# sebcossu/yocto_raytracing

Measured on AMD Instinct MI355X. Metric: Mrays/sec + ms/frame, instance10000 1920×1080×64spp, 1/2/4/8 MI355X, higher is better.
Workload: dtype f32; 1 GPU; instance10000 1920x1080 8x8 spp, amb 0.1, one frame per step; scene=instance10000, width=1920, height=1080, spp=64, parallelism=single GPU, algorithm=wavefront

## Files before the change

__graft_entry__.py:

```python
from __future__ import annotations

import ctypes
import importlib
import sys
from pathlib import Path

ROOT = Path(__file__).resolve().parent
if str(ROOT) not in sys.path:
    sys.path.insert(0, str(ROOT))


def _build_module():
    import importlib.util

    spec = importlib.util.spec_from_file_location("yrt_build", ROOT / "yocto_raytracing_amd" / "build.py")
    mod = importlib.util.module_from_spec(spec)
    spec.loader.exec_module(mod)
    return mod


def _variants_tool():
    import importlib.util

    spec = importlib.util.spec_from_file_location("yrt_build_variants", ROOT / "tools" / "build_variants.py")
    mod = importlib.util.module_from_spec(spec)
    spec.loader.exec_module(mod)
    return mod


def build() -> None:
    b = _build_module()
    b.build_library()
    b.build_oracle()
    t = _variants_tool()
    t.main(t.test_specs(), default_library=False, verbose=False)
    importlib.import_module("yocto_raytracing_amd")


def _oracle():
    lib = ctypes.CDLL(str(ROOT / "oracle" / "liboracle.so"))
    lib.oracle_load.restype = ctypes.c_void_p
    lib.oracle_load.argtypes = [ctypes.c_char_p]
    lib.oracle_render_rows.restype = ctypes.c_longlong
    lib.oracle_render_rows.argtypes = [ctypes.c_void_p, ctypes.c_float, ctypes.c_int, ctypes.c_int,
                                       ctypes.c_int, ctypes.c_int, ctypes.c_int, ctypes.c_void_p,
                                       ctypes.c_int, ctypes.c_int, ctypes.c_int, ctypes.c_void_p,
                                       ctypes.c_void_p]
    return lib


def smoke() -> None:
    import numpy as np

    import yocto_raytracing_amd as yrt

    if yrt.device_count() < 1:
        raise RuntimeError("smoke: no GPU visible")
    scene_path = ROOT / "tests" / "golden" / "scenes" / "simple.yrtscene"
    scn = yrt.load_scene(str(scene_path))
    yrt.build_bvh(scn)
    res, s = 36, 2
    img, stats = yrt.raytrace(scn, (0.1, 0.1, 0.1), res, s, return_stats=True)

    lib = _oracle()
    o = lib.oracle_load(str(scene_path).encode())
    h, w = img.shape[:2]
    rows = np.arange(h, dtype=np.int32)
    ref = np.zeros_like(img)
    nrays = lib.oracle_render_rows(o, 0.1, 0, res, 0, s, 16, rows.ctypes.data, h, 0, w, ref.ctypes.data, None)
    diff = float(np.abs(img - ref).max())
    exact = float(np.mean(img.view(np.uint32) == ref.view(np.uint32)))
    if stats["rays"] != nrays or diff > 1e-5:
        raise RuntimeError(f"smoke: GPU/oracle mismatch rays {stats['rays']} vs {nrays}, max|diff| {diff}")
    print(f"smoke ok: {w}x{h}x{s * s} rays={nrays} bit-exact={exact:.4f} max|diff|={diff:.3g}")


if __name__ == "__main__":
    build()
    smoke()
```

yocto_raytracing_amd/csrc/wavefront.hip:

```cpp
#include <hip/hip_runtime.h>

#include <algorithm>
#include <cstdio>
#include <cstdlib>
#include <cstring>
#include <stdexcept>
#include <type_traits>

#include "item_magic.h"
#include "packet_trace.h"
#include "trace_common.h"
#include "wf_workspace.h"
#include "yrt_render.h"

namespace yrt {
namespace {

constexpr int WF_BLOCK = 256;
#ifndef YRT_PRIMARY_BLOCK
#define YRT_PRIMARY_BLOCK 64
#endif
#ifndef YRT_SHADOW_BLOCK
#define YRT_SHADOW_BLOCK 64
#endif
// ... 1920 lines not shown
                vec3f v;
                float vlen;
                normalize_len(ro - p, v, vlen);
                for (int li = 0; li < S.nlights; li++) {
                    if (OCC4 ? ((occ_bits >> li) & 1u) != 0u : ldb(B.occl + (size_t)li * B.capacity + idx) != 0) continue;
                    const f4* lr = S.lights + 6 * li;
                    float4 lrec[6];
                    ld_scalar<6>(lr, lrec);
                    frame3f lf = {xyz(lrec[0]), xyz(lrec[1]), xyz(lrec[2]), xyz(lrec[3])};
                    vec3f lp0 = xyz(lrec[4]), ke = xyz(lrec[5]);
                    vec3f tp = transform_point(lf, lp0 - p);
                    vec3f l, h;
                    float r, hlen;
                    normalize_len(tp, l, r);
                    normalize_len(v + l, h, hlen);
                    vec3f kd = kd0, ks = ks0;
                    if (kd_txt >= 0) kd = kd * tkd;
                    if (ks_txt >= 0) ks = ks * tks;
                    const vec3f ker = div3(ke, r * r);
                    vec3f ld = kd * ker;
                    vec3f ls = ks * ker;
                    if (kind == kind_lines) {
                        float prodnl = dot(nrm, l);
                        float prodnh = dot(nrm, h);
                        if (prodnl < 0.0f) prodnl *= -1;
                        if (prodnh < 0.0f) prodnh *= -1;
                        float sinnl = __builtin_sqrtf(1.0f - prodnl);
                        float sinnh = __builtin_sqrtf(1.0f - prodnh);
                        ld = ld * sinnl;
                        ls = ls * spec_pow(sinnh, ns, ls);
                    } else {
                        ld = ld * smax(0.0f, dot(nrm, l));
                        ls = ls * spec_pow(smax(0.0f, dot(nrm, h)), ns, ls);
                    }
                    c = c + (ld + ls);
                    cd = cd + ld;
                    cs = cs + ls;
                }
                pc = c, pd = cd, ps = cs, pla = la;
                if (!reflective) {
                    R = c + la;
                } else {
                    truncated++;
                    vec3f t = {0.0f * kr.x, 0.0f * kr.y, 0.0f * kr.z};
                    pr = t;
                    R = (c + t) + la;
                }
            }
        }
        if constexpr (FUSE) {
            auto put = [&](int k, const vec3f& val) {
                if (!(P.mask >> k & 1)) return;
                fused[(k * 3 + 0) * ROW + threadIdx.x] = val.x;
                fused[(k * 3 + 1) * ROW + threadIdx.x] = val.y;
                fused[(k * 3 + 2) * ROW + threadIdx.x] = val.z;
            };
            put(pass_direct, pc), put(pass_diffuse, pd), put(pass_specular, ps);
            put(pass_reflection, pr), put(pass_ambient, pla), put(pass_count, R);
            continue;
        }
    }
    }
    if (FUSE) {
        __syncthreads();
        const int ppb = SB / C.spp;
        for (int t = (int)threadIdx.x; t < 3 * pass_planes * ppb; t += SB) {
            const int px = t / (3 * pass_planes), r = t - 3 * pass_planes * px;
            const int k = r / 3, comp = r - 3 * k;
            if (!(P.mask >> k & 1)) continue;
            const int pl = (int)(blockIdx.x * SB / C.spp) + px;
            int lx, ly, i, j;
            const bool valid = pl < C.npix && pixel_of(A, C, C.pix0 + pl, lx, ly, i, j);
            if (pl < C.npix && lx < A.tile_w && ly < A.tile_h) {
                float v = 0.0f;
                if (valid) {
                    const float* row = fused + (k * 3 + comp) * ROW + px * C.spp;
                    float acc = 0.0f;
                    for (int q = 0; q < C.spp; q++) acc = acc + row[q];
                    v = acc / float(C.spp);
                }
                float* o = reinterpret_cast<float*>(P.out[k] + (size_t)ly * A.out_stride + lx);
                o[comp] = v;
                if (comp == 0) o[3] = valid ? 1.0f : 0.0f;
            }
        }
    }
    flush(counters, cnt_depth_truncated, truncated);
}

struct group_buffers {
    int nplanes;
    unsigned amb_mask;
    const int* tab;
    float4* out[group_planes];
    f4* smp[group_planes];
    f4* rec[group_planes];
};

constexpr int shade_group_waves = 5;
template <bool FUSE, int SB = WF_BLOCK, bool OCC4 = false>
__global__ __launch_bounds__(SB, shade_group_waves) void k_shade_groups(dev_scene_view S, dev_render_args A, int level,
                                                                        int nsamp_level0, int max_depth, wf_buffers B,
                                                                        group_buffers G, unsigned long long* counters,
                                                                        chunk_args C) {
    constexpr int ROW = SB + 1;
    __shared__ float fused[FUSE ? group_planes * 3 * ROW : 1];
    __shared__ int cmp_count[SB / 64], cmp_base[SB / 64];
    __shared__ srgb_table srgb_lds;
    const float* lut = stage_srgb<SB, true>(S, srgb_lds);
    work_counts wc;
    unsigned long long truncated = 0;
    float amb_x = A.amb[0], amb_y = A.amb[1], amb_z = A.amb[2];
    float cam_x = A.cam.ox, cam_y = A.cam.oy, cam_z = A.cam.oz;
    asm volatile("" : "+s"(amb_x), "+s"(amb_y), "+s"(amb_z), "+s"(cam_x), "+s"(cam_y), "+s"(cam_z));
    const vec3f amb = {amb_x, amb_y, amb_z};
    const vec3f cam_o = {cam_x, cam_y, cam_z};
    const int nplanes = G.nplanes;
    const int* order = G.tab + group_planes + 1;
    const int stride = gridDim.x * SB;
    const int gout = (int)(blockIdx.x % (unsigned)level_segments);
    const int nseg = FUSE ? 1 : level ? level_segments : 1;
    for (int g = 0; g < nseg; g++) {
    const int n = (!FUSE && level) ? *seg_counter(B.count, level, g) : nsamp_level0;
    const int nround = (n + stride - 1) / stride;
    for (int round = 0; round < nround; round++) {
        const int j = round * stride + blockIdx.x * SB + threadIdx.x;
        const int idx = FUSE ? j : g * B.seg + j;
        bool hit = false, write_r = false, spawn = false, reflective = false;
        vec3f p = {0, 0, 0}, nrm = {0, 0, 0}, v = {0, 0, 0}, dr = {0, 0, 0};
        vec3f kd = {0, 0, 0}, ks = {0, 0, 0}, kr = {0, 0, 0}, la = {0, 0, 0}, la0 = {0, 0, 0}, t = {0, 0, 0};
        float ns = 0.0f;
        int mat = 0, kind = 0;
        uint32_t occ_bits = 0;
        if (j < n) {
            const float4 s0 = ld4s(B.surf0 + idx);
            if constexpr (OCC4) {
#pragma unroll
                for (int q = 0; q < 4; q++) {
                    const int lq = q < S.nlights ? q : 0;
                    occ_bits |= (ldb(B.occl + (size_t)lq * B.capacity + idx) != 0u ? 1u : 0u) << q;
                }
            }
            const int info = sample_state(s0);
            write_r = info != -2;
            hit = info >= 0;
            if (hit) {
                const float4 ro4 =
                    (!FUSE && level) ? ld4(B.ray_o(level) + idx) : make_float4(cam_o.x, cam_o.y, cam_o.z, 0.0f);
                vec2f uv;
                {
                    const float4 s1 = ld4s(B.surf1 + idx);
                    p = xyz(s0), nrm = xyz(s1), uv = {s1.w, B.need_v ? lds1(B.surfv + idx) : 0.0f};
                    mat = info_mat(info), kind = info & 3;
                }
                const vec3f ro = xyz(ro4);
                const float4 m0 = ld4(S.mats + 4 * mat), m1 = ld4(S.mats + 4 * mat + 1);
                const float4 m2 = ld4(S.mats + 4 * mat + 2), m3 = ld4(S.mats + 4 * mat + 3);
                const vec3f kd0 = xyz(m0), ks0 = xyz(m1);
                kr = xyz(m2), ns = m0.w;
                const int kd_txt = ibits(m1.w), ks_txt = ibits(m2.w);
                reflective = ibits(m3.w) & mat_reflective;
                const vec3f zero = {0.0f, 0.0f, 0.0f};
                la = amb * kd0, la0 = zero * kd0;
                vec3f tkd = {1, 1, 1}, tks = {1, 1, 1};
                if (kd_txt >= 0) {
                    tkd = eval_texture<false>(S, kd_txt, uv, wc, lut);
                    la = la * tkd, la0 = la0 * tkd;
                }
                if (ks_txt >= 0) tks = eval_texture<false>(S, ks_txt, uv, wc, lut);
                kd = kd0, ks = ks0;
                if (kd_txt >= 0) kd = kd * tkd;
                if (ks_txt >= 0) ks = ks * tks;
                float vlen;
                normalize_len(ro - p, v, vlen);
                if (reflective) {
                    if (FUSE || level + 1 >= max_depth || level + 1 >= B.nlevels) {
                        truncated++;
                        t = {0.0f * kr.x, 0.0f * kr.y, 0.0f * kr.z};
                    } else {
                        spawn = true;
                        dr = (nrm * 2.0f * dot(nrm, v)) - v;
                        write_r = false;
                    }
                }
            }
        }
        for (int k = 0; k < nplanes; k++) {
            const int q0 = __builtin_amdgcn_readfirstlane(G.tab[k]), q1 = __builtin_amdgcn_readfirstlane(G.tab[k + 1]);
            const bool ambk = G.amb_mask >> k & 1;
            vec3f R = {0, 0, 0};
            if (hit) {
                vec3f c = {0.0f, 0.0f, 0.0f};
                for (int q = q0; q < q1; q++) {
                    const int li = __builtin_amdgcn_readfirstlane(order[q]);
                    if (OCC4 ? ((occ_bits >> li) & 1u) != 0u : ldb(B.occl + (size_t)li * B.capacity + idx) != 0) continue;
                    float4 lrec[6];
                    ld_scalar<6>(S.lights + 6 * li, lrec);
                    frame3f lf = {xyz(lrec[0]), xyz(lrec[1]), xyz(lrec[2]), xyz(lrec[3])};
                    vec3f lp0 = xyz(lrec[4]), ke = xyz(lrec[5]);
                    vec3f tp = transform_point(lf, lp0 - p);
                    vec3f l, h;
                    float r, hlen;
                    normalize_len(tp, l, r);
                    normalize_len(v + l, h, hlen);
                    const vec3f ker = div3(ke, r * r);
                    vec3f ld = kd * ker;
                    vec3f ls = ks * ker;
                    if (kind == kind_lines) {
                        float prodnl = dot(nrm, l);
                        float prodnh = dot(nrm, h);
                        if (prodnl < 0.0f) prodnl *= -1;
                        if (prodnh < 0.0f) prodnh *= -1;
                        float sinnl = __builtin_sqrtf(1.0f - prodnl);
                        float sinnh = __builtin_sqrtf(1.0f - prodnh);
                        ld = ld * sinnl;
                        ls = ls * spec_pow(sinnh, ns, ls);
                    } else {
                        ld = ld * smax(0.0f, dot(nrm, l));
                        ls = ls * spec_pow(smax(0.0f, dot(nrm, h)), ns, ls);
                    }
                    c = c + (ld + ls);
                }
                const vec3f lak = ambk ? la : la0;
                if (!reflective)
                    R = c + lak;
                else if (!spawn)
                    R = (c + t) + lak;
                else
                    G.rec[k][(size_t)level * B.capacity + idx] = {c.x, c.y, c.z, __int_as_float(mat)};
            }
            if constexpr (FUSE) {
                fused[(k * 3 + 0) * ROW + threadIdx.x] = R.x;
                fused[(k * 3 + 1) * ROW + threadIdx.x] = R.y;
                fused[(k * 3 + 2) * ROW + threadIdx.x] = R.z;
            } else if (write_r) {
                vec3f col = R;
                int lev = level, node = idx;
                while (lev > 0) {
                    const int parent = ibits(B.ray_o(lev)[node].w);
                    const float4 d = ld4(G.rec[k] + (size_t)(lev - 1) * B.capacity + parent);
                    const float4 pkr = ld4(S.mats + 4 * ibits(d.w) + 2);
                    vec3f cc = {d.x, d.y, d.z};
                    const vec3f tt = {col.x * pkr.x, col.y * pkr.y, col.z * pkr.z};
                    cc = cc + tt;
                    if (ambk) cc = cc + xyz(ld4(B.rec1(lev - 1) + parent));
                    col = cc, node = parent, lev--;
                }
                G.smp[k][node] = {col.x, col.y, col.z, 1.0f};
            }
        }
        if constexpr (FUSE) continue;
        const unsigned long long mask = __ballot(spawn);
        const int w = threadIdx.x >> 6, lane = threadIdx.x & 63;
        if (spawn) B.rec1(level)[idx] = {la.x, la.y, la.z, 0};
        if (lane == 0) cmp_count[w] = __popcll(mask);
        __syncthreads();
        if (threadIdx.x == 0) {
            int tot = 0;
            for (int q = 0; q < SB / 64; q++) tot += cmp_count[q];
            int acc = tot ? atomicAdd(seg_counter(B.count, level + 1, gout), tot) : 0;
            for (int q = 0; q < SB / 64; q++) cmp_base[q] = acc, acc += cmp_count[q];
        }
        __syncthreads();
        if (spawn) {
            const int slot = gout * B.seg + cmp_base[w] + __popcll(mask & ((1ull << lane) - 1));
            B.ray_o(level + 1)[slot] = {p.x, p.y, p.z, __int_as_float(idx)};
            B.ray_d(level + 1)[slot] = {dr.x, dr.y, dr.z, 0};
        }
    }
    }
    if (FUSE) {
        __syncthreads();
        const int ppb = SB / C.spp;
        for (int e = (int)threadIdx.x; e < 3 * nplanes * ppb; e += SB) {
            const int px = e / (3 * nplanes), r = e - 3 * nplanes * px;
            const int k = r / 3, comp = r - 3 * k;
            const int pl = (int)(blockIdx.x * SB / C.spp) + px;
            int lx, ly, i, j;
            const bool valid = pl < C.npix && pixel_of(A, C, C.pix0 + pl, lx, ly, i, j);
            if (pl < C.npix && lx < A.tile_w && ly < A.tile_h) {
                float val = 0.0f;
                if (valid) {
                    const float* row = fused + (k * 3 + comp) * ROW + px * C.spp;
                    float acc = 0.0f;
                    for (int q = 0; q < C.spp; q++) acc = acc + row[q];
                    val = acc / float(C.spp);
                }
                float* o = reinterpret_cast<float*>(G.out[k] + (size_t)ly * A.out_stride + lx);
                o[comp] = val;
                if (comp == 0) o[3] = valid ? 1.0f : 0.0f;
            }
        }
    }
    flush(counters, cnt_depth_truncated, truncated);
}

#if !defined(YRT_SHADOW_SHADE_FUSE)
#define YRT_SHADOW_SHADE_FUSE 1
#endif
#define YRT_SHADOW_SHADE_KERNEL (YRT_SHADOW_SHADE_FUSE && YRT_SHADOW_ITEM_LIGHTS)
#if !defined(YRT_LIGHT_CARRY)
#define YRT_LIGHT_CARRY 1
#endif
#if (YRT_SHADOW_SHADE_KERNEL)
__global__ __launch_bounds__(SP_BLOCK, YRT_SHADOW_WAVES) void k_shadow_shade_persist(dev_scene_view S,
                                                                                      dev_render_args A, int nsamp,
                                                                                      int nx, wf_buffers B,
                                                                                      unsigned long long* counters,
                                                                                      chunk_args C,
                                                                                      float4* __restrict__ out) {
    constexpr int WPB = SP_BLOCK / 64;
    constexpr unsigned RUN = YRT_SHADOW_ITEM_RUN;
    constexpr int CARRY = YRT_LIGHT_CARRY ? 4 : 0;
    __shared__ float4 wave_slab[WPB][CARRY ? CARRY : 1][64];
    __shared__ unsigned wave_truncated[WPB];
    __shared__ srgb_table srgb_lds;
    __shared__ struct {
        dev_render_args A;
        chunk_args C;
    } args;
    const float* lut = stage_srgb<SP_BLOCK, false>(S, srgb_lds);
    if (threadIdx.x == 0) args.A = A, args.C = C;
    __syncthreads();
    float cam_x = A.cam.ox, cam_y = A.cam.oy, cam_z = A.cam.oz;
    asm volatile("" : "+s"(cam_x), "+s"(cam_y), "+s"(cam_z));
    const vec3f cam_o = {cam_x, cam_y, cam_z};
    const int nl = S.nlights;
    __builtin_assume(nl > 0);
    const unsigned n_items = (unsigned)nx;
    auto lane_now = []() {
        unsigned l;
        asm volatile("v_mbcnt_lo_u32_b32 %0, -1, 0\n\tv_mbcnt_hi_u32_b32 %0, -1, %0" : "=v"(l));
        return l;
    };
    const int w = __builtin_amdgcn_readfirstlane((int)(threadIdx.x >> 6));
    const unsigned xcd = blockIdx.x % 8u;
    unsigned rays = 0, culled = 0;
    if (lane_now() == 0) wave_truncated[w] = 0;
    constexpr unsigned CS = YRT_SHADOW_BLOCK_CHUNK;
    __shared__ chunk_ring ring;
    const unsigned head = head_items<RUN, CS>(n_items);
    chunk_ring_init<CS>(ring, B.queue + xcd, B.queue + 8, head / 8u);
    for (;;) {
        const unsigned q = chunk_ring_next<CS>(ring, B.queue + xcd, lane_now(), B.queue + 8, head / 8u);
        const unsigned it = split_item<RUN>(q, xcd, n_items, head);
        if (it >= n_items) break;
        const int bx = (int)it;
        uint32_t occ_bits = 0;
        for (int li = 0; li < nl; li++) {
            bool valid;
            const bool occ = shadow_item_light<0, true, true>(S, B, nsamp, bx, li, nl, lane_now(), cam_o, nullptr, rays,
                                                              culled, valid, li < CARRY ? wave_slab[w][li] : nullptr);
            occ_bits |= (occ ? 1u : 0u) << li;
        }
        const int idx = bx * 64 + (int)lane_now();
        vec3f R = {0, 0, 0};
        unsigned long long truncated = 0;
        if (idx < nsamp) {
            const float4 s0 = ld4(B.surf0 + idx);
            const int info = sample_state(s0);
            if (info >= 0) {
                const float4 ro4 = make_float4(cam_o.x, cam_o.y, cam_o.z, 0.0f);
                const float* amb = args.A.amb;
                work_counts wc;
                vec3f p = {0, 0, 0}, dr = {0, 0, 0}, rec_d = {0, 0, 0}, rec_la = {0, 0, 0};
                int rec_mat = 0;
                bool spawn = false, write_r = true;
                shade_hit<false, true, true, true>(S, B, idx, info, s0, ro4, occ_bits, 0, 1, amb, lut, wc, truncated, R, p,
                                             spawn, dr, rec_d, rec_la, rec_mat, write_r, (no_terms*)nullptr,
                                             CARRY ? &wave_slab[w][0][lane_now()] : nullptr, CARRY);
            }
        }
        const unsigned lane = lane_now();
        const unsigned ntrunc = (unsigned)__popcll(ballot(truncated != 0));
        if (ntrunc && lane == 0) wave_truncated[w] += ntrunc;
        wave_slab[w][0][lane] = make_float4(R.x, R.y, R.z, 1.0f);
        asm volatile("s_waitcnt lgkmcnt(0)" ::: "memory");
        const int spp = __builtin_amdgcn_readfirstlane(args.C.spp);
        if (spp == 64) {
            sum_pixels<64, 64>(args.A, args.C, out, wave_slab[w][0], bx, 1, (int)lane);
        } else {
            const int sl = __builtin_ctz((unsigned)spp);
            sum_pixels<64>(args.A, args.C, out, wave_slab[w][0], bx << (6 - sl), 64 >> sl, (int)lane);
        }
        asm volatile("s_waitcnt lgkmcnt(0)" ::: "memory");
    }
    const unsigned lane = lane_now();
    const unsigned long long first = lane == 0 ? 1ull : 0ull;
    flush_block_at<3, SP_BLOCK>(
        counters, {first * rays, first * culled, first * (lane == 0 ? wave_truncated[w] : 0u)},
        (unsigned)w * 64u + lane,
        [](unsigned k) { return k == 0 ? cnt_shadow_rays : k == 1 ? cnt_shadow_culled : cnt_depth_truncated; });
}
#endif

constexpr int AQ = 8;
template <class SMP, class OUT>
__device__ __forceinline__ void accumulate_plane(dev_render_args A, chunk_args C, SMP&& samples, OUT&& out) {
    __shared__ float4 stage[WF_BLOCK / 64][64 * (AQ + 1)];
    const int w = threadIdx.x >> 6, lane = threadIdx.x & 63;
    const int pl0 = blockIdx.x * WF_BLOCK + w * 64;
    const int np = max(0, min(64, C.npix - pl0));
    float4* S = stage[w];
    const f4* base = samples() + (size_t)pl0 * C.spp;
    vec3f acc = {0, 0, 0};
    for (int q0 = 0; q0 < C.spp; q0 += AQ) {
        const int qn = min(AQ, C.spp - q0);
        for (int e = lane; e < np * qn; e += 64) {
            const int px = e / qn, q = e % qn;
            S[px * (AQ + 1) + q] = ld4(base + (size_t)px * C.spp + q0 + q);
        }
        __syncthreads();
        if (lane < np)
            for (int q = 0; q < qn; q++) {
                const float4 c = S[lane * (AQ + 1) + q];
                acc = {acc.x + c.x, acc.y + c.y, acc.z + c.z};
            }
        __syncthreads();
    }
    if (lane >= np) return;
    const int pl = pl0 + lane;
    int lx, ly, i, j;
    const bool valid = pixel_of(A, C, C.pix0 + pl, lx, ly, i, j);
    if (lx >= A.tile_w || ly >= A.tile_h) return;
    const float d = float(C.spp);
    out()[(size_t)ly * A.out_stride + lx] =
        valid ? make_float4(acc.x / d, acc.y / d, acc.z / d, 1.0f) : make_float4(0.0f, 0.0f, 0.0f, 0.0f);
}

__global__ __launch_bounds__(WF_BLOCK) void k_accumulate(dev_render_args A, chunk_args C, wf_buffers B,
                                                         float4* __restrict__ out) {
    accumulate_plane(A, C, [&] { return B.rad; }, [&] { return out; });
}

__global__ __launch_bounds__(WF_BLOCK) void k_accumulate_passes(dev_render_args A, chunk_args C, wf_buffers B,
                                                                pass_buffers P) {
    const int k = (int)blockIdx.y;
    if (!(P.mask >> k & 1)) return;
    accumulate_plane(A, C, [&] { return k == pass_count ? B.rad : P.smp[k]; }, [&] { return P.out[k]; });
}

__global__ __launch_bounds__(WF_BLOCK) void k_accumulate_groups(dev_render_args A, chunk_args C, group_buffers G) {
    const int k = (int)blockIdx.y;
    accumulate_plane(A, C, [&] { return G.smp[k]; }, [&] { return G.out[k]; });
}

wf_buffers carve(void* base, const workspace_shape& s, pass_buffers* P, group_buffers* G) {
    wf_buffers B = {};
    workspace_carver w(base);
    int pass = -1;
    walk_workspace(s, [&](wf_slab slab, int k, size_t bytes) {
        void* const p = w.take(bytes);
        switch (slab) {
            case slab_count: B.count = (int*)p; break;
            case slab_queue: B.queue = (unsigned*)p; break;
            case slab_lstats: B.lstats = (unsigned long long*)p; break;
            case slab_surf0: B.surf0 = (f4*)p; break;
            case slab_surf1: B.surf1 = (f4*)p; break;
            case slab_surfv: B.surfv = (float*)p; break;
            case slab_occl: B.occl = (unsigned char*)p; break;
            case slab_rad: B.rad = (f4*)p; break;
            case slab_pbox: B.pbox = (f4*)p; break;
            case slab_lcount: B.lcount = (int*)p; break;
            case slab_lskip: B.lskip = (int*)p; break;
            case slab_lists: B.lists = (f4*)p; break;
            case slab_slists: B.slists = (f4*)p; break;
            case slab_ccount: B.ccount = (int*)p; break;
            case slab_cskip: B.cskip = (int*)p; break;
            case slab_clist: B.clist = (f4*)p; break;
            case slab_ray_o: B.ray_o_ = (f4*)p; break;
            case slab_ray_d: B.ray_d_ = (f4*)p; break;
            case slab_rec0: B.rec0_ = (f4*)p; break;
            case slab_rec1: B.rec1_ = (f4*)p; break;
            case slab_pass_smp:
                do pass++;
                while (!(P->mask >> pass & 1));
                P->smp[pass] = (f4*)p;
                break;
            case slab_group_tab: G->tab = (const int*)p; break;
            case slab_group_smp: G->smp[k] = (f4*)p; break;
            case slab_group_rec: G->rec[k] = (f4*)p; break;
        }
    });
    if (G) G->smp[0] = B.rad, G->rec[0] = B.rec0_;
    B.capacity = s.cap;
    B.nlevels = s.nlevels;
    return B;
}


hipError_t clear_counters(unsigned long long* counters, hipStream_t stream) {
    return counters ? hipMemsetAsync(counters, 0, (size_t)cnt_slots * cnt_count * sizeof(unsigned long long), stream)
                    : hipSuccess;
}

template <class F>
long long chunk_target(const device_scene& ds, const dev_render_args& A, F&& bytes_of) {
    long long target = 1ll << (ds.reflective ? MIRROR_CHUNK_LOG2 : CHUNK_LOG2);
    if (bytes_of(target) > ds.work_bytes) {
        size_t free_b = 0, total_b = 0;
        if (hipMemGetInfo(&free_b, &total_b) != hipSuccess) free_b = 0;
        free_b += ds.work_bytes;
        while (target > (1ll << 16) && bytes_of(target) > free_b / 2) target /= 2;
        if (bytes_of(target) > free_b)
            throw unsupported_error("max_depth " + std::to_string(A.max_depth) + " needs " +
                                    std::to_string(bytes_of(target) >> 20) + " MiB of mirror-level records for its " +
                                    "smallest chunk; " + std::to_string(free_b >> 20) + " MiB of HBM are free");
    }
    return target;
}

hipError_t grow_workspace(device_scene& ds, size_t need) {
    if (need <= ds.work_bytes) return hipSuccess;
    if (ds.work) (void)hipFree(ds.work);
    ds.work = nullptr;
    ds.work_bytes = 0;
    hipError_t e = hipMalloc(&ds.work, need);
    if (e == hipSuccess) ds.work_bytes = need;
    return e;
}

hipError_t make_level_counts(device_scene& ds) {
    if (!ds.level_count_host) {
        hipError_t e = hipHostMalloc((void**)&ds.level_count_host, sizeof(int) * level_segments * count_stride,
                                     hipHostMallocDefault);
        if (e != hipSuccess) return e;
    }
    if (!ds.level_count_ev) return hipEventCreateWithFlags(&ds.level_count_ev, hipEventDisableTiming);
    return hipSuccess;
}
hipError_t make_list_stats(device_scene& ds) {
    if (!ds.list_stats_host) {
        hipError_t e =
            hipHostMalloc((void**)&ds.list_stats_host, list_sums * sizeof(unsigned long long), hipHostMallocDefault);
        if (e != hipSuccess) return e;
        memset(ds.list_stats_host, 0, list_sums * sizeof(unsigned long long));
    }
    if (!ds.list_stats_ev) return hipEventCreateWithFlags(&ds.list_stats_ev, hipEventDisableTiming);
    return hipSuccess;
}
hipError_t fetch_level_counts(device_scene& ds, const wf_buffers& B, int level, hipStream_t stream) {
    hipError_t e = hipMemcpyAsync(ds.level_count_host, B.count + (size_t)level * level_segments * count_stride,
                                  sizeof(int) * level_segments * count_stride, hipMemcpyDeviceToHost, stream);
    return e == hipSuccess ? hipEventRecord(ds.level_count_ev, stream) : e;
}
hipError_t level_has_rays(device_scene& ds, bool& any) {
    hipError_t e = hipEventSynchronize(ds.level_count_ev);
    any = false;
    for (int g = 0; e == hipSuccess && g < level_segments; g++) any |= ds.level_count_host[g * count_stride] != 0;
    return e;
}

void launch_chunk_setup(const device_scene& ds, const wf_buffers& B, int nrec, const float4& cam4,
                        unsigned long long* lstats, int nlevels, unsigned long long* counters, bool first_chunk,
                        hipStream_t stream) {
    const int count_ints = nlevels > 1 ? (int)(count_bytes(nlevels) / sizeof(int)) : 0;
    const int counter_words = first_chunk && counters ? cnt_slots * cnt_count : 0;
    const int work = std::max(std::max(nrec, count_ints), std::max(counter_words, 32));
    const int nb = std::min((work + WF_BLOCK - 1) / WF_BLOCK, 1024);
    hipLaunchKernelGGL(k_chunk_setup, dim3(nb), dim3(WF_BLOCK), 0, stream, nrec ? ds.view.tpair : nullptr, nrec,
                       cam4.x, cam4.y, cam4.z, ds.trel, B.queue, lstats, B.count, count_ints, counters,
                       counter_words);
}

struct chunk_plan {
    int nlevels;
    bool fuse;
    int per_chunk;
    int seg, cap;
    wf_buffers B;
};
hipError_t plan_chunks(device_scene& ds, const dev_render_args& A, long long units, int granule, int spp,
                       pass_buffers* P, group_buffers* G, chunk_plan& plan) {
    const int nlevels = plan.nlevels = ds.reflective ? std::max(A.max_depth, 1) : 1;
    const bool fuse = plan.fuse = nlevels == 1 && WF_BLOCK % spp == 0;
    const int smp_planes = P && !fuse ? __builtin_popcount(P->mask & ((1u << pass_count) - 1)) : 0;
    auto units_for = [&](long long tgt) {
        const int u = (int)std::max<long long>(1, std::min<long long>(units, tgt / spp));
        return (u + granule - 1) / granule * granule;
    };
    auto seg_of = [&](int u) { return u * spp / level_segments + level_segments * WF_BLOCK; };
    auto cap_of = [&](int u) { return nlevels > 1 ? level_segments * seg_of(u) : u * spp; };
    auto shape_of = [&](int u) {
        const size_t samples = (size_t)u * spp;
        return workspace_shape{cap_of(u), spp, ds.nlights, nlevels, smp_planes, samples,
                               G ? G->nplanes : 0, fuse ? 0 : samples};
    };
    plan.per_chunk =
        units_for(chunk_target(ds, A, [&](long long tgt) { return workspace_bytes(shape_of(units_for(tgt))); }));
    plan.seg = seg_of(plan.per_chunk);
    plan.cap = cap_of(plan.per_chunk);
    const workspace_shape shape = shape_of(plan.per_chunk);
    if (hipError_t e = grow_workspace(ds, workspace_bytes(shape)); e != hipSuccess) return e;
    plan.B = carve(ds.work, shape, P, G);
    plan.B.seg = plan.seg;
    plan.B.need_v = ds.view.ntextures > 0;
    return nlevels > 1 ? make_level_counts(ds) : hipSuccess;
}

template <class F>
decltype(auto) with_bool(bool b, F&& f) {
    return b ? f(std::true_type()) : f(std::false_type());
}

template <class F>
hipError_t with_walk(const device_scene& ds, bool packet, F&& f) {
    if (packet) return f(std::true_type(), uint32_t());
    if (ds.narrow_stack) return f(std::false_type(), uint16_t());
    return f(std::false_type(), uint32_t());
}

constexpr int stride_grid = 2048;

template <bool COUNT, bool PACKET, typename SE, class SHADOW0, class SHADE>
hipError_t run_levels(device_scene& ds, const wf_buffers& B, int nlevels, int nsamp, const float4& cam4,
                      unsigned long long* counters, hipStream_t stream, SHADOW0&& shadow0, bool level0_shaded,
                      SHADE&& shade) {
    phase_timer& T = ds.timer;
    constexpr int TB = shadow_block<PACKET>();
    for (int level = 0; level < nlevels; level++) {
        if (level > 0) {
            int t = T.begin(phase_bounce, stream);
            hipLaunchKernelGGL((k_bounce<COUNT, PACKET, SE>), dim3(stride_grid), dim3(WF_BLOCK), 0, stream, ds.view,
                               level, B, counters);
            T.end(t, stream);
            bool any;
            if (hipError_t e = level_has_rays(ds, any); e != hipSuccess) return e;
            if (!any) break;
        }
        if (ds.nlights > 0) {
            int t = T.begin(phase_shadow, stream);
            if (level > 0 || !shadow0()) {
                const dim3 sg(level ? stride_grid * WF_BLOCK / TB : (nsamp + TB - 1) / TB, ds.nlights);
                with_bool(!COUNT && PACKET && ds.wide_ok, [&](auto wide) {
                    hipLaunchKernelGGL((k_shadow<COUNT, PACKET, SE, decltype(wide)::value>), sg, dim3(TB), 0, stream,
                                       ds.view, level, nsamp, B, counters, cam4);
                });
            }
            T.end(t, stream);
        }
        if (level == 0 && level0_shaded) continue;
        int t = T.begin(phase_shade, stream);
        shade(level, dim3(level ? stride_grid : (nsamp + WF_BLOCK - 1) / WF_BLOCK));
        T.end(t, stream);
        if (level + 1 < nlevels) {
            if (hipError_t e = fetch_level_counts(ds, B, level + 1, stream); e != hipSuccess) return e;
        }
    }
    return hipSuccess;
}

template <bool COUNT, bool PACKET, typename SE>
hipError_t run(device_scene& ds, const dev_render_args& A, float4* out, unsigned long long* counters,
               hipStream_t stream, const pass_buffers* passes = nullptr, const group_buffers* groups = nullptr) {
    const int spp = A.samples * A.samples;
    const int tiles_x = (A.tile_w + TILE - 1) / TILE;
    const int tiles_y = (A.tile_h + TILE - 1) / TILE;
    const long long npix_total = (long long)tiles_x * tiles_y * TILE * TILE;
    pass_buffers P = passes ? *passes : pass_buffers{};
    group_buffers G = groups ? *groups : group_buffers{};
    chunk_plan plan;
    if (hipError_t e = plan_chunks(ds, A, npix_total, TILE * TILE, spp, passes ? &P : nullptr,
// ... 342 lines not shown
```

Measured before the change: 34310 Mrays/s.

## Park surface sample in LDS and split light culling from occlusion tracing

In the fused shadow+shade persistent kernel, each wave now loads surf0/surf1 once per item and parks surf0 in an LDS slab row. It runs a separate pass computing light directions and the zero-term culling for all lights, then a second loop traces any-hit rays reusing the parked sample and the carried directions. Shading reads the parked sample from LDS instead of reloading it from global memory. The aim is to cut repeated global loads of surface data and to skip tracing early when a light is culled for the whole wave. The cost is one fewer carry row for light directions (3 instead of 4), so more lights recompute their direction, plus extra LDS traffic and code complexity. The build entry also switches from test_specs to build_specs.

```diff
diff --git a/__graft_entry__.py b/__graft_entry__.py
--- a/__graft_entry__.py
+++ b/__graft_entry__.py
@@ -33,7 +33,7 @@
     b.build_library()
     b.build_oracle()
     t = _variants_tool()
-    t.main(t.test_specs(), default_library=False, verbose=False)
+    t.main(t.build_specs(), default_library=False, verbose=False)
     importlib.import_module("yocto_raytracing_amd")
 
 
diff --git a/yocto_raytracing_amd/csrc/wavefront.hip b/yocto_raytracing_amd/csrc/wavefront.hip
--- a/yocto_raytracing_amd/csrc/wavefront.hip
+++ b/yocto_raytracing_amd/csrc/wavefront.hip
@@ -2246,6 +2246,9 @@
 #if !defined(YRT_LIGHT_CARRY)
 #define YRT_LIGHT_CARRY 1
 #endif
+#if !defined(YRT_SURF_PARK)
+#define YRT_SURF_PARK 1
+#endif
 #if (YRT_SHADOW_SHADE_KERNEL)
 __global__ __launch_bounds__(SP_BLOCK, YRT_SHADOW_WAVES) void k_shadow_shade_persist(dev_scene_view S,
                                                                                       dev_render_args A, int nsamp,
@@ -2255,8 +2258,10 @@
                                                                                       float4* __restrict__ out) {
     constexpr int WPB = SP_BLOCK / 64;
     constexpr unsigned RUN = YRT_SHADOW_ITEM_RUN;
-    constexpr int CARRY = YRT_LIGHT_CARRY ? 4 : 0;
-    __shared__ float4 wave_slab[WPB][CARRY ? CARRY : 1][64];
+    constexpr bool PARK = YRT_SURF_PARK && YRT_LIGHT_CARRY;
+    constexpr int ROWS = YRT_LIGHT_CARRY ? 4 : 1;
+    constexpr int CARRY = YRT_LIGHT_CARRY ? ROWS - (PARK ? 1 : 0) : 0;
+    __shared__ float4 wave_slab[WPB][ROWS][64];
     __shared__ unsigned wave_truncated[WPB];
     __shared__ srgb_table srgb_lds;
     __shared__ struct {
@@ -2291,17 +2296,100 @@
         if (it >= n_items) break;
         const int bx = (int)it;
         uint32_t occ_bits = 0;
+#if (YRT_SURF_PARK && YRT_LIGHT_CARRY)
+        {
+            const unsigned lane = lane_now();
+            const int idx = bx * 64 + (int)lane;
+            int info = -1;
+            float4 s0 = {0, 0, 0, __int_as_float(-1)}, s1 = {0, 0, 0, 0};
+            static_assert(bundle_max_lights <= 24, "occ_bits: the lights' bits below the count's byte");
+            int lcl = -1;
+            if (B.bundles && (int)lane < nl) lcl = B.lcount[(bx / bundle_g) * nl + (int)lane];
+            if (idx < nsamp) {
+                s0 = ld4(B.surf0 + idx);
+                s1 = ld4(B.surf1 + idx);
+                info = sample_state(s0);
+            }
+            if (B.bundles) occ_bits = (uint32_t)lcl << 24;
+            wave_slab[w][CARRY][lane] = s0;
+            const bool valid = info >= 0;
+#pragma nounroll
+            for (int li = 0; li < nl; li++) {
+                float4 lrec[6];
+                ld_records_at<6>(S.lights, (unsigned)(6 * li), lrec);
+                const frame3f lf = {xyz(lrec[0]), xyz(lrec[1]), xyz(lrec[2]), xyz(lrec[3])};
+                const vec3f lp0 = xyz(lrec[4]);
+                float r = 1.0f;
+                vec3f o = {0, 0, 0}, d = {0, 0, 1};
+                if (valid) {
+                    const vec3f p = xyz(s0);
+                    vec3f tp = transform_point(lf, lp0 - p);
+                    vec3f l;
+                    normalize_len(tp, l, r);
+                    o = p, d = l;
+                    if (li < CARRY) wave_slab[w][li][lane] = make_float4(l.x, l.y, l.z, r);
+                }
+                rays += (unsigned)__popcll(ballot(valid));
+                const bool zero_term = light_term_zero(info, xyz(s1), o, cam_o, d, r, xyz(lrec[5]));
+                culled += (unsigned)__popcll(ballot(zero_term));
+                occ_bits |= (zero_term ? 1u : 0u) << li;
+            }
+        }
+#pragma nounroll
+        for (int li = 0; li < nl; li++) {
+            const unsigned lane = lane_now();
+            const float4 s0 = wave_slab[w][CARRY][lane];
+            const bool valid = sample_state(s0) >= 0;
+            const unsigned long long cull = ballot(((occ_bits >> li) & 1u) != 0u);
+            if (cull == ballot(valid)) continue;
+            int lc = -1;
+            if (B.bundles) lc = __builtin_amdgcn_readlane((int)occ_bits, li) >> 24;
+            if (lc == 0) continue;
+            const f4* tbase = S.wnodes;
+            uint32_t troot = (uint32_t)S.wtop_root;
+            if (lc > 0) {
+                tbase = B.lists;
+                troot = (uint32_t)(((bx / bundle_g) * nl + li) * bundle_recs * wide_record_bytes);
+            }
+            vec3f l = {0, 0, 1};
+            float r = 1.0f;
+            if (li < CARRY) {
+                if (valid) {
+                    const float4 c4 = wave_slab[w][li][lane];
+                    l = xyz(c4), r = c4.w;
+                }
+            } else {
+                float4 lrec[5];
+                ld_records_at<5>(S.lights, (unsigned)(6 * li), lrec);
+                const frame3f lf = {xyz(lrec[0]), xyz(lrec[1]), xyz(lrec[2]), xyz(lrec[3])};
+                if (valid) {
+                    vec3f tp = transform_point(lf, xyz(lrec[4]) - xyz(s0));
+                    normalize_len(tp, l, r);
+                }
+            }
+            ray3 sr = {{0, 0, 0}, {0, 0, 1}, 0.01f, 1.0f};
+            if (valid) sr = {xyz(s0), l, 0.01f, r - 0.01f};
+            const bool occ = item_any_hit<0>(S, sr, valid, nullptr, tbase, troot, cull);
+            occ_bits |= (occ ? 1u : 0u) << li;
+        }
+        if (B.bundles) occ_bits &= 0xffffffu;
+#else
         for (int li = 0; li < nl; li++) {
             bool valid;
             const bool occ = shadow_item_light<0, true, true>(S, B, nsamp, bx, li, nl, lane_now(), cam_o, nullptr, rays,
                                                               culled, valid, li < CARRY ? wave_slab[w][li] : nullptr);
             occ_bits |= (occ ? 1u : 0u) << li;
         }
+#endif
         const int idx = bx * 64 + (int)lane_now();
         vec3f R = {0, 0, 0};
         unsigned long long truncated = 0;
         if (idx < nsamp) {
+#if (YRT_SURF_PARK && YRT_LIGHT_CARRY)
+            const float4 s0 = wave_slab[w][CARRY][lane_now()];
+#else
             const float4 s0 = ld4(B.surf0 + idx);
+#endif
             const int info = sample_state(s0);
             if (info >= 0) {
                 const float4 ro4 = make_float4(cam_o.x, cam_o.y, cam_o.z, 0.0f);
```

Result: no change. 34580 Mrays/s (median of 6 runs) (+0.8%).
